# srndpty/kobato-eyes

Measured on AMD Instinct MI355X. Metric: images/s (pHash + all-pairs Hamming scan + cluster membership), higher is better.
Workload: dtype u8 luma, int32 taps (i8 matrix cores), f64 DCT, 1-bit Hamming products (fp4 matrix cores, exact)

## Files before the change

kobato-eyes_amd/csrc/ke_hash.hip:

```cpp
#include <cstdlib>

#include "ke_internal.h"
#include "dct_table.h"
#include "ke_hash_select.h"
#include "ke_resample_plan.h"

namespace {

constexpr int kPrecisionBits = 22;

__device__ __forceinline__ int clip8_fixed(int acc) {
    int v = acc >> kPrecisionBits;
    return v < 0 ? 0 : (v > 255 ? 255 : v);
}

__device__ __forceinline__ int luma_of(const uint8_t *p, int ch) {
    if (ch == 1) return p[0];
    return (int)((19595u * p[0] + 38470u * p[1] + 7471u * p[2] + 0x8000u) >> 16);
}

template <int AXIS>
__global__ __launch_bounds__(256) void ke_resample_pass(const uint8_t *__restrict__ src,
                                                         const uint64_t *__restrict__ offsets, uint64_t stride,
                                                         int ch, int w, int h, const int32_t *__restrict__ bounds,
                                                         const int32_t *__restrict__ kk, int ksize, int out_size,
                                                         uint8_t *__restrict__ dst, int blocks_per_image) {
    const int64_t img = blockIdx.x / blocks_per_image;
    const int blk = blockIdx.x % blocks_per_image;
    const int ow = AXIS == 0 ? out_size : w;
    const int oh = AXIS == 0 ? h : out_size;
    const int e = blk * 256 + threadIdx.x;
    if (e >= ow * oh) return;
    const int oy = e / ow, ox = e % ow;
    const uint8_t *base = src + (offsets ? offsets[img] : (uint64_t)img * stride);
    const int o = AXIS == 0 ? ox : oy;
    const int first = bounds[2 * o], cnt = bounds[2 * o + 1];
    const int32_t *k = kk + (size_t)o * ksize;
    int acc = 1 << (kPrecisionBits - 1);
    if (AXIS == 0) {
        const uint8_t *row = base + ((size_t)oy * w + first) * ch;
        for (int t = 0; t < cnt; ++t) acc += luma_of(row + (size_t)t * ch, ch) * k[t];
    } else {
        const uint8_t *col = base + ((size_t)first * w + ox) * ch;
        for (int t = 0; t < cnt; ++t) acc += luma_of(col + (size_t)t * w * ch, ch) * k[t];
    }
    dst[(size_t)img * ow * oh + e] = (uint8_t)clip8_fixed(acc);
}

__constant__ double c_C32[4][16];
__constant__ double c_C16[2][8];
__constant__ double c_C8[4];

__device__ double dct32_one(const double *x, int k) {
    if (k & 1) {
        const int q = k >> 1;
        double acc = 0.0;
#pragma unroll
        for (int n = 0; n < 16; ++n) acc = fma(x[n] - x[31 - n], c_C32[q][n], acc);
        return acc;
    }
    double u[16];
#pragma unroll
    for (int n = 0; n < 16; ++n) u[n] = x[n] + x[31 - n];
    if (k & 2) {
        const int q = k >> 2;
        double acc = 0.0;
#pragma unroll
        for (int n = 0; n < 8; ++n) acc = fma(u[n] - u[15 - n], c_C16[q][n], acc);
        return acc;
    }
    double v[8];
#pragma unroll
    for (int n = 0; n < 8; ++n) v[n] = u[n] + u[15 - n];
    if (k == 4) {
        double acc = 0.0;
#pragma unroll
        for (int n = 0; n < 4; ++n) acc = fma(v[n] - v[7 - n], c_C8[n], acc);
        return acc;
    }
    const double w0 = v[0] + v[7], w1 = v[1] + v[6], w2 = v[2] + v[5], w3 = v[3] + v[4];
    return (w0 + w1) + (w2 + w3);
}

__device__ uint64_t tile32_to_phash(const uint8_t *tile, double *Td, float *cf, int tid, float *margin = nullptr) {
    {
        const int y = tid >> 3, kx = tid & 7;
        double x[32];
#pragma unroll
        for (int n = 0; n < 32; ++n) x[n] = (double)tile[y * 32 + n];
        Td[y * 8 + kx] = dct32_one(x, kx);
    }
    __syncthreads();
    if (tid < 64) {
        const int ky = tid >> 3, kx = tid & 7;
        double x[32];
#pragma unroll
        for (int n = 0; n < 32; ++n) x[n] = Td[n * 8 + kx];
        const double s = (ky == 0 && kx == 0) ? KE_SCALE00 : ((ky == 0 || kx == 0) ? KE_SCALE0K : KE_SCALEKK);
        cf[tid] = (float)(dct32_one(x, ky) * s);
    }
    __syncthreads();
    uint64_t hash = 0;
    if (tid < 64) {
        const float *a = cf + 1;
        float r[8];
#pragma unroll
        for (int j = 0; j < 8; ++j) r[j] = a[j];
#pragma unroll
        for (int i = 8; i < 56; i += 8)
#pragma unroll
            for (int j = 0; j < 8; ++j) r[j] = r[j] + a[i + j];
        float res = ((r[0] + r[1]) + (r[2] + r[3])) + ((r[4] + r[5]) + (r[6] + r[7]));
#pragma unroll
        for (int i = 56; i < 63; ++i) res = res + a[i];
        const float mean = res / 63.0f;
        const unsigned long long m = __ballot(cf[tid] > mean);
        hash = __brevll(m);
        if (margin) {
            float mg = fabsf(cf[tid] - mean);
#pragma unroll
            for (int s = 32; s > 0; s >>= 1) mg = fminf(mg, __shfl_xor(mg, s));
            if (tid == 0) *margin = mg;
        }
    }
    return hash;
}

__global__ __launch_bounds__(256) void ke_tiles_to_hashes(const uint8_t *__restrict__ tile32,
                                                           const uint8_t *__restrict__ tile98,
                                                           const int64_t *__restrict__ out_idx,
                                                           uint64_t *__restrict__ phash, uint64_t *__restrict__ dhash,
                                                           float *__restrict__ margin) {
    __shared__ __attribute__((aligned(16))) uint8_t s_tile[1024];
    __shared__ double s_T[256];
    __shared__ float s_cf[64];
    const int tid = threadIdx.x;
    const int64_t img = blockIdx.x;
    const int64_t slot = out_idx ? out_idx[img] : img;
    if (phash) {
        reinterpret_cast<uint32_t *>(s_tile)[tid] = reinterpret_cast<const uint32_t *>(tile32 + (size_t)img * 1024)[tid];
        __syncthreads();
        const uint64_t hv = tile32_to_phash(s_tile, s_T, s_cf, tid, margin ? margin + slot : nullptr);
        if (tid == 0) phash[slot] = hv;
    }
    if (dhash && tid < 64) {
        const uint8_t *t = tile98 + (size_t)img * 72;
        const int r = tid >> 3, c = tid & 7;
        const unsigned long long m = __ballot(t[r * 9 + c + 1] > t[r * 9 + c]);
        if (tid == 0) dhash[slot] = __brevll(m);
    }
}

template <bool kTransposed>
__device__ __forceinline__ void tile32_coeffs(const uint8_t *tile, double *Td, float *cf, int tid) {
    {
        const int y = tid >> 3, kx = tid & 7;
        double x[32];
#pragma unroll
        for (int n = 0; n < 32; ++n) x[n] = (double)tile[kTransposed ? n * 32 + y : y * 32 + n];
        Td[y * 8 + kx] = dct32_one(x, kx);
    }
    __syncthreads();
    if (tid < 64) {
        const int ky = tid >> 3, kx = tid & 7;
        double x[32];
#pragma unroll
        for (int n = 0; n < 32; ++n) x[n] = Td[n * 8 + kx];
        const double s = (ky == 0 && kx == 0) ? KE_SCALE00 : ((ky == 0 || kx == 0) ? KE_SCALE0K : KE_SCALEKK);
        cf[tid] = (float)(dct32_one(x, ky) * s);
    }
    __syncthreads();
}

__global__ __launch_bounds__(256) void ke_tiles_to_phash_turned(const uint8_t *__restrict__ tile32, const int64_t *__restrict__ out_idx,
                                                                 uint64_t *__restrict__ turned) {
    __shared__ __attribute__((aligned(16))) uint8_t s_tile[1024];
    __shared__ double s_T[256];
    __shared__ float s_cf[2][64];
    const int tid = threadIdx.x, lane = tid & 63, wv = tid >> 6;
    const int64_t img = blockIdx.x;
    const int64_t slot = out_idx ? out_idx[img] : img;
    reinterpret_cast<uint32_t *>(s_tile)[tid] = reinterpret_cast<const uint32_t *>(tile32 + (size_t)img * 1024)[tid];
    __syncthreads();
    tile32_coeffs<false>(s_tile, s_T, s_cf[0], tid);
// ... 15 lines not shown
#pragma unroll
        for (int i = 56; i < 63; ++i) res = res + coef(1 + i);
        const float mean = res / 63.0f;
        const unsigned long long m = __ballot(coef(lane) > mean);
        if (lane == 0) turned[slot * 8 + k] = __brevll(m);
    }
}

__device__ __forceinline__ uint32_t luma4_biased(uint32_t d0, uint32_t d1, uint32_t d2) {
    constexpr uint32_t CHI = 0x001D964Cu, CLO = 0x002F468Bu, START = 0x8000u - 0x800000u;
    const uint32_t p0 = d0;
    const uint32_t p1 = __builtin_amdgcn_alignbyte(d1, d0, 3);
    const uint32_t p2 = __builtin_amdgcn_alignbyte(d2, d1, 2);
    const uint32_t s0 = (__builtin_amdgcn_udot4(p0, CHI, 0u, false) << 8) + __builtin_amdgcn_udot4(p0, CLO, START, false);
    const uint32_t s1 = (__builtin_amdgcn_udot4(p1, CHI, 0u, false) << 8) + __builtin_amdgcn_udot4(p1, CLO, START, false);
    const uint32_t s2 = (__builtin_amdgcn_udot4(p2, CHI, 0u, false) << 8) + __builtin_amdgcn_udot4(p2, CLO, START, false);
    const uint32_t s3 = (__builtin_amdgcn_udot4(d2, CHI << 8, 0u, false) << 8) + __builtin_amdgcn_udot4(d2, CLO << 8, START, false);
    const uint32_t lo = __builtin_amdgcn_perm(s1, s0, 0x0C0C0602u);
    const uint32_t hi = __builtin_amdgcn_perm(s3, s2, 0x06020C0Cu);
    return lo | hi;
}

template <int C>
__device__ __forceinline__ uint32_t luma4_generic(const uint32_t *d) {
    if (C == 3) return luma4_biased(d[0], d[1], d[2]);
    if (C == 1) return d[0] ^ 0x80808080u;
    constexpr uint32_t CHI = 0x001D964Cu, CLO = 0x002F468Bu, START = 0x8000u - 0x800000u;
    uint32_t s[4];
#pragma unroll
    for (int k = 0; k < 4; ++k)
        s[k] = (__builtin_amdgcn_udot4(d[k], CHI, 0u, false) << 8) + __builtin_amdgcn_udot4(d[k], CLO, START, false);
    return __builtin_amdgcn_perm(s[1], s[0], 0x0C0C0602u) | __builtin_amdgcn_perm(s[3], s[2], 0x06020C0Cu);
}

__device__ __forceinline__ int combine_planes(int d0, int d1, int d2, int bias) {
    return (int)((uint32_t)d0 + ((uint32_t)d1 << 8) + ((uint32_t)d2 << 16) + (uint32_t)bias);
}

struct KeFusedArgs {
    const uint8_t *pixels;
    const uint64_t *offsets;
    uint64_t stride;
    const int64_t *out_idx;
    int h;
    const int32_t *mx_frag;
    int mx_base0, mx_base1;
    const int32_t *h_bias;
    const int32_t *v_packed, *v_start, *v_bias;
    int ndwv;
    int qw, qw_inv, lp;
    int w, row_bytes;
    int lt_half;
    int lt_bytes;
    int hp;
    uint64_t *phash;
    float *margin;
    uint8_t *tile32_out;
    const int32_t *mxd_frag, *hd_bias;
    const int32_t *vd_cpacked, *vd_cstart, *vd_bias;
    int ndwcv;
    int hpd;
    int x_off;
    int bands, band_rows;
    uint8_t *hs, *hsd;
    int hs_hp, hsd_hp;
    uint64_t *dhash;
    uint8_t *tile98_out;
};

template <int C>
__device__ __forceinline__ void patch_last_quad(const uint8_t *image_last_row, int w, uint8_t *lds_row) {
    for (int x = w & ~3; x < w; ++x) lds_row[x] = (uint8_t)(luma_of(image_last_row + (size_t)x * C, C) ^ 0x80);
}

__device__ __forceinline__ void band_writeout(const uint8_t *HT, int hp, int ncols, int rows, uint8_t *dst, int dst_hp, int tid,
                                              int nthreads) {
    const int wpc = (rows + 3) / 4;
    for (int e = tid; e < ncols * wpc; e += nthreads) {
        const int col = e / wpc, k = e % wpc;
        *reinterpret_cast<uint32_t *>(dst + (size_t)col * dst_hp + 4 * k) = *reinterpret_cast<const uint32_t *>(HT + col * hp + 4 * k);
    }
}

template <int NDWD>
__device__ __forceinline__ void fused_tail(const KeFusedArgs &a, uint8_t *Lt, const uint8_t *HT, const uint8_t *HTd,
                                           const int tid, const int64_t img) {
    uint8_t *T32 = Lt;
    double *Td = reinterpret_cast<double *>(Lt + 1024);
    float *cf = reinterpret_cast<float *>(Lt + 1024 + 2048);
    {
        const int yy = tid & 31, og = tid >> 5;
        const int rotv = (yy >> 4) & 1;
        const int vst = a.v_start[yy];
        const int ndwv = a.ndwv;
        int acc[4][3];
#pragma unroll
        for (int m = 0; m < 4; ++m) acc[m][0] = acc[m][1] = acc[m][2] = 0;
        for (int j = 0; j < ndwv; j += 2) {
            const int jj = j ^ (2 * rotv);
            const int32_t *cp = a.v_packed + ((size_t)yy * ndwv + jj) * 3;
            const int c00 = cp[0], c01 = cp[1], c02 = cp[2], c10 = cp[3], c11 = cp[4], c12 = cp[5];
#pragma unroll
            for (int m = 0; m < 4; ++m) {
                const uint2 v = *reinterpret_cast<const uint2 *>(
                    __builtin_assume_aligned(HT + (size_t)(og + 8 * m) * a.hp + vst + 4 * jj, 8));
                acc[m][0] = __builtin_amdgcn_sdot4((int)v.x, c00, acc[m][0], false);
                acc[m][1] = __builtin_amdgcn_sdot4((int)v.x, c01, acc[m][1], false);
                acc[m][2] = __builtin_amdgcn_sdot4((int)v.x, c02, acc[m][2], false);
                acc[m][0] = __builtin_amdgcn_sdot4((int)v.y, c10, acc[m][0], false);
                acc[m][1] = __builtin_amdgcn_sdot4((int)v.y, c11, acc[m][1], false);
                acc[m][2] = __builtin_amdgcn_sdot4((int)v.y, c12, acc[m][2], false);
            }
        }
        const int vbias = a.v_bias[yy];
#pragma unroll
        for (int m = 0; m < 4; ++m)
            T32[yy * 32 + og + 8 * m] = (uint8_t)clip8_fixed(combine_planes(acc[m][0], acc[m][1], acc[m][2], vbias));
    }
    __syncthreads();
    if (a.tile32_out)
        reinterpret_cast<uint32_t *>(a.tile32_out + (size_t)img * 1024)[tid] = reinterpret_cast<const uint32_t *>(T32)[tid];
    const int64_t slot = a.out_idx ? a.out_idx[img] : img;
    const uint64_t hv = tile32_to_phash(T32, Td, cf, tid, (a.margin && a.phash) ? a.margin + slot : nullptr);
    if (tid == 0 && a.phash) a.phash[slot] = hv;
    if (NDWD > 0) {
        __syncthreads();
        int *part = reinterpret_cast<int *>(Lt);
        uint8_t *T98 = Lt + 1024;
        if (tid < 216) {
            const int out = tid / 3, chunk = tid % 3;
            const int yy = out / 9, oc = out % 9;
            const int vc = yy * 3 + chunk;
            const int vst = a.vd_cstart[vc];
            const int nd = a.ndwcv;
            int d0 = 0, d1 = 0, d2 = 0;
            for (int j = 0; j < nd; j += 2) {
                const int32_t *cp = a.vd_cpacked + ((size_t)vc * nd + j) * 3;
                const uint2 v = *reinterpret_cast<const uint2 *>(__builtin_assume_aligned(HTd + (size_t)oc * a.hpd + vst + 4 * j, 8));
                d0 = __builtin_amdgcn_sdot4((int)v.x, cp[0], d0, false);
                d1 = __builtin_amdgcn_sdot4((int)v.x, cp[1], d1, false);
                d2 = __builtin_amdgcn_sdot4((int)v.x, cp[2], d2, false);
                d0 = __builtin_amdgcn_sdot4((int)v.y, cp[3], d0, false);
                d1 = __builtin_amdgcn_sdot4((int)v.y, cp[4], d1, false);
                d2 = __builtin_amdgcn_sdot4((int)v.y, cp[5], d2, false);
            }
            part[tid] = combine_planes(d0, d1, d2, 0);
        }
        __syncthreads();
        if (tid < 72) {
            const int yy = tid / 9;
            const uint32_t sum = (uint32_t)part[3 * tid] + (uint32_t)part[3 * tid + 1] + (uint32_t)part[3 * tid + 2] + (uint32_t)a.vd_bias[yy];
            T98[tid] = (uint8_t)clip8_fixed((int)sum);
        }
        __syncthreads();
        if (a.tile98_out && tid < 72) a.tile98_out[(size_t)img * 72 + tid] = T98[tid];
        if (tid < 64) {
            const int r = tid >> 3, c = tid & 7;
            const unsigned long long m = __ballot(T98[r * 9 + c + 1] > T98[r * 9 + c]);
            if (tid == 0 && a.dhash) a.dhash[a.out_idx ? a.out_idx[img] : img] = __brevll(m);
        }
    }
}

int upload_dct_tables(ke_ctx *ctx) {
    if (ctx->dct_tables_ready) return KE_OK;
    KE_HIP(ctx, hipMemcpyToSymbol(HIP_SYMBOL(c_C32), KE_C32, sizeof(KE_C32)));
    KE_HIP(ctx, hipMemcpyToSymbol(HIP_SYMBOL(c_C16), KE_C16, sizeof(KE_C16)));
    KE_HIP(ctx, hipMemcpyToSymbol(HIP_SYMBOL(c_C8), KE_C8, sizeof(KE_C8)));
    ctx->dct_tables_ready = true;
    return KE_OK;
}

constexpr int kRTM = kKeTileRowsMx;
typedef int ke_v4i __attribute__((ext_vector_type(4)));

template <int W64, int KS, bool DH, bool GEN, int C, bool UNAL>
__global__ __launch_bounds__(256, 2) void ke_phash_fused_mx(const KeFusedArgs a) {
    static_assert(!UNAL || GEN, "rows that are not a multiple of 4 pixels need the run-time row length");
    constexpr uint32_t QB = 4u * C;
    constexpr int W = 64 * W64;
    constexpr int QPT = kRTM * (W / 4) / 256;
    const int QW = GEN ? a.qw : W / 4;
    const int QUADS_PER_TILE = kRTM * QW;
    const int LP = GEN ? a.lp : W + 16;
    constexpr int KD = (W64 + 1) / 2;
    extern __shared__ __attribute__((aligned(16))) uint8_t smem[];
    uint8_t *Lt = smem;
    uint8_t *HT = smem + a.lt_bytes;
    uint8_t *HTd = HT + 32 * a.hp;
    uint8_t *X = smem + a.x_off;
    const int tid = threadIdx.x;
    const int lane = tid & 63, wv = tid >> 6;
    const int64_t img = a.bands ? blockIdx.x / a.bands : blockIdx.x;
    const int y_begin = a.bands ? (int)(blockIdx.x % a.bands) * a.band_rows : 0;
    const uint32_t row_bytes = UNAL ? (uint32_t)a.row_bytes : (uint32_t)QW * QB;
    const uint8_t *src = a.pixels + (a.offsets ? a.offsets[img] : (uint64_t)img * a.stride) + (size_t)y_begin * row_bytes;
    const int h = a.bands ? min(a.band_rows, a.h - y_begin) : a.h;
    const uint32_t image_bytes = (uint32_t)(a.h - y_begin) * row_bytes;

    const int mt = wv >> 1, jt = wv & 1;
    ke_v4i bf[KS][3];
#pragma unroll
    for (int s = 0; s < KS; ++s)
#pragma unroll
        for (int p = 0; p < 3; ++p)
            bf[s][p] = reinterpret_cast<const ke_v4i *>(a.mx_frag)[((jt * KS + s) * 3 + p) * 64 + lane];
    constexpr int KDR = DH ? KD : 1;
    ke_v4i bd[KDR][3];
    int dbias = 0;
    if (DH) {
#pragma unroll
        for (int d = 0; d < KDR; ++d)
#pragma unroll
            for (int p = 0; p < 3; ++p)
                bd[d][p] = reinterpret_cast<const ke_v4i *>(a.mxd_frag)[((jt * KD + d) * 3 + p) * 64 + lane];
        dbias = a.hd_bias[(lane & 15) < 9 ? (lane & 15) : 8];
    }
    const int ocol = 16 * jt + (lane & 15);
    const int hbias = a.h_bias[ocol];
    const int a_off = (16 * mt + (lane & 15)) * LP + (jt ? a.mx_base1 : a.mx_base0) + 16 * (lane >> 4);
    const int d_off = (16 * mt + (lane & 15)) * LP + 64 * KD * jt + 16 * (lane >> 4);
    uint8_t *ht_dst = HT + (size_t)ocol * a.hp + 16 * mt + 4 * (lane >> 4);
    uint8_t *htd_dst = HTd + (size_t)(lane & 15) * a.hpd + 16 * mt + 4 * (lane >> 4);
    ke_v4i *x_slot = reinterpret_cast<ke_v4i *>(X + mt * 1024 + lane * 16);

    uint32_t raw[QPT][C];
    auto load_tile = [&](int t) {
        const uint32_t tile_off = UNAL ? (uint32_t)t * (kRTM * row_bytes) : (uint32_t)t * ((uint32_t)QUADS_PER_TILE * QB);
        const uint8_t *tile_ptr = src + tile_off;
        const uint32_t lim = UNAL ? image_bytes - QB - tile_off : min(image_bytes - QB - tile_off, (uint32_t)(QUADS_PER_TILE - 1) * QB);
#pragma unroll
        for (int q = 0; q < QPT; ++q) {
            uint32_t vo = (uint32_t)(q * 256 + tid) * QB;
            if (UNAL) {
                const uint32_t i = min((uint32_t)(q * 256 + tid), (uint32_t)(QUADS_PER_TILE - 1));
                const uint32_t row = __umulhi(i, (uint32_t)a.qw_inv);
                vo = row * row_bytes + (i - row * (uint32_t)QW) * QB;
            }
            const uint32_t off = vo < lim ? vo : lim;
            const uint32_t *p = reinterpret_cast<const uint32_t *>(tile_ptr + off);
#pragma unroll
            for (int k = 0; k < C; ++k) raw[q][k] = __builtin_nontemporal_load(p + k);
        }
    };
    auto store_luma = [&](uint8_t *dst) {
#pragma unroll
        for (int q = 0; q < QPT; ++q) {
            const int i = q * 256 + tid;
            if (GEN) {
                const int row = (int)__umulhi((uint32_t)i, (uint32_t)a.qw_inv);
                if (i < QUADS_PER_TILE)
                    *reinterpret_cast<uint32_t *>(dst + row * LP + (i - row * QW) * 4) = luma4_generic<C>(raw[q]);
            } else {
                *reinterpret_cast<uint32_t *>(dst + (i / (W / 4)) * LP + (i % (W / 4)) * 4) = luma4_generic<C>(raw[q]);
            }
        }
    };
    auto pack_rows = [](const ke_v4i &v0, const ke_v4i &v1, const ke_v4i &v2, int bias) {
        uint32_t packed = 0;
#pragma unroll
        for (int i = 0; i < 4; ++i) packed |= (uint32_t)clip8_fixed(combine_planes(v0[i], v1[i], v2[i], bias)) << (8 * i);
        return packed ^ 0x80808080u;
    };
    auto products = [&](int t, const uint8_t *cur) -> ke_v4i {
        ke_v4i acc[3], dacc[3];
#pragma unroll
        for (int p = 0; p < 3; ++p) acc[p] = dacc[p] = ke_v4i{0, 0, 0, 0};
        const uint8_t *ap = cur + a_off;
#pragma unroll
        for (int s = 0; s < KS; ++s) {
            const ke_v4i av = *reinterpret_cast<const ke_v4i *>(__builtin_assume_aligned(ap + 64 * s, 16));
#pragma unroll
            for (int p = 0; p < 3; ++p) acc[p] = __builtin_amdgcn_mfma_i32_16x16x64_i8(av, bf[s][p], acc[p], 0, 0, 0);
        }
        if (DH) {
            const uint8_t *dp = cur + d_off;
#pragma unroll
            for (int d = 0; d < KDR; ++d) {
                const ke_v4i av = *reinterpret_cast<const ke_v4i *>(__builtin_assume_aligned(dp + 64 * d, 16));
#pragma unroll
                for (int p = 0; p < 3; ++p) dacc[p] = __builtin_amdgcn_mfma_i32_16x16x64_i8(av, bd[d][p], dacc[p], 0, 0, 0);
            }
        }
        *reinterpret_cast<uint32_t *>(ht_dst + t * kRTM) = pack_rows(acc[0], acc[1], acc[2], hbias);
        ke_v4i part;
#pragma unroll
        for (int i = 0; i < 4; ++i) part[i] = combine_planes(dacc[0][i], dacc[1][i], dacc[2][i], 0);
        return part;
    };
    ke_v4i carry = {0, 0, 0, 0};
    auto finish_dhash = [&](int t) {
        const ke_v4i other = x_slot[(t & 1) * 128];
        const ke_v4i zero = {0, 0, 0, 0};
        const ke_v4i sum = carry + other;
        const uint32_t packed = pack_rows(sum, zero, zero, dbias);
        if ((lane & 15) < 9) *reinterpret_cast<uint32_t *>(htd_dst + t * kRTM) = packed;
    };
    auto hpass = [&](int t, const uint8_t *cur) {
        if (!DH) {
            products(t, cur);
        } else if (jt) {
            x_slot[(t & 1) * 128] = products(t, cur);
        } else {
            if (t > 0) finish_dhash(t - 1);
            carry = products(t, cur);
        }
    };

    const int ntiles = (h + kRTM - 1) / kRTM;
    load_tile(0);
    store_luma(Lt);
    __syncthreads();
    for (int t = 0; t + 1 < ntiles; ++t) {
        load_tile(t + 1);
        __builtin_amdgcn_sched_barrier(0);
        hpass(t, Lt + (t & 1) * a.lt_half);
        __builtin_amdgcn_sched_barrier(0);
        store_luma(Lt + ((t + 1) & 1) * a.lt_half);
        __syncthreads();
    }
    if (UNAL) {
        if (tid == 0 && y_begin + h == a.h)
            patch_last_quad<C>(src + (size_t)(h - 1) * row_bytes, a.w, Lt + ((ntiles - 1) & 1) * a.lt_half + ((h - 1) - (ntiles - 1) * kRTM) * LP);
        __syncthreads();
    }
    hpass(ntiles - 1, Lt + ((ntiles - 1) & 1) * a.lt_half);
    __syncthreads();
    if (DH) {
        if (!jt) finish_dhash(ntiles - 1);
        __syncthreads();
    }
    if (a.bands) {
        band_writeout(HT, a.hp, 32, h, a.hs + (size_t)img * 32 * a.hs_hp + y_begin, a.hs_hp, tid, 256);
        if (DH) band_writeout(HTd, a.hpd, 9, h, a.hsd + (size_t)img * 9 * a.hsd_hp + y_begin, a.hsd_hp, tid, 256);
        return;
    }
    fused_tail<(DH ? 1 : 0)>(a, Lt, HT, HTd, tid, img);
}

constexpr int kRTW = kKeTileRowsWide;

template <int KSH, int QPT, bool DH, int KDW, int C, bool UNAL>
__global__ __launch_bounds__(512, 1) void ke_phash_fused_wide(const KeFusedArgs a) {
    constexpr uint32_t QB = 4u * C;
    extern __shared__ __attribute__((aligned(16))) uint8_t smem[];
    uint8_t *Lt = smem;
    uint8_t *HT = smem + a.lt_bytes;
    uint8_t *HTd = HT + 32 * a.hp;
    uint8_t *X = smem + a.x_off;
    const int tid = threadIdx.x;
    const int lane = tid & 63, wv = tid >> 6;
    const int jt = wv & 1, kh = wv >> 1;
    const int64_t img = a.bands ? blockIdx.x / a.bands : blockIdx.x;
    const int y_begin = a.bands ? (int)(blockIdx.x % a.bands) * a.band_rows : 0;
    const int QW = a.qw, LP = a.lp;
    const uint32_t row_bytes = UNAL ? (uint32_t)a.row_bytes : (uint32_t)QW * QB;
    const uint8_t *src = a.pixels + (a.offsets ? a.offsets[img] : (uint64_t)img * a.stride) + (size_t)y_begin * row_bytes;
    const int h = a.bands ? min(a.band_rows, a.h - y_begin) : a.h;
    const int quads_per_tile = kRTW * QW;
    const uint32_t image_bytes = (uint32_t)(a.h - y_begin) * row_bytes;

    ke_v4i bf[KSH][3];
#pragma unroll
    for (int s = 0; s < KSH; ++s)
#pragma unroll
        for (int p = 0; p < 3; ++p)
            bf[s][p] = reinterpret_cast<const ke_v4i *>(a.mx_frag)[((jt * 4 * KSH + kh * KSH + s) * 3 + p) * 64 + lane];
    const int ocol = 16 * jt + (lane & 15);
    const int hbias = a.h_bias[ocol];
    const int a_off = (lane & 15) * LP + (jt ? a.mx_base1 : a.mx_base0) + 64 * KSH * kh + 16 * (lane >> 4);
    uint8_t *ht_dst = HT + (size_t)ocol * a.hp + 4 * (lane >> 4);
    ke_v4i *x_slot = reinterpret_cast<ke_v4i *>(X) + jt * 192 + lane;
    constexpr int KDR = DH ? KDW : 1;
    ke_v4i bd[KDR][3];
    int dbias = 0;
    if (DH) {
#pragma unroll
        for (int d = 0; d < KDR; ++d)
#pragma unroll
            for (int p = 0; p < 3; ++p)
                bd[d][p] = reinterpret_cast<const ke_v4i *>(a.mxd_frag)[((wv * KDW + d) * 3 + p) * 64 + lane];
        dbias = a.hd_bias[(lane & 15) < 9 ? (lane & 15) : 8];
    }
    const int d_off = (lane & 15) * LP + 64 * KDW * wv + 16 * (lane >> 4);
    uint8_t *htd_dst = HTd + (size_t)(lane & 15) * a.hpd + 4 * (lane >> 4);
    ke_v4i *xd_slot = reinterpret_cast<ke_v4i *>(X) + 768 + lane;

    uint32_t raw[QPT][C];
    auto load_tile = [&](int t) {
        const uint32_t tile_off = UNAL ? (uint32_t)t * (kRTW * row_bytes) : (uint32_t)t * ((uint32_t)quads_per_tile * QB);
        const uint8_t *tile_ptr = src + tile_off;
        const uint32_t lim = UNAL ? image_bytes - QB - tile_off : min(image_bytes - QB - tile_off, (uint32_t)(quads_per_tile - 1) * QB);
#pragma unroll
        for (int q = 0; q < QPT; ++q) {
            uint32_t vo = (uint32_t)(q * 512 + tid) * QB;
            if (UNAL) {
                const uint32_t i = min((uint32_t)(q * 512 + tid), (uint32_t)(quads_per_tile - 1));
                const uint32_t row = __umulhi(i, (uint32_t)a.qw_inv);
                vo = row * row_bytes + (i - row * (uint32_t)QW) * QB;
            }
            const uint32_t off = vo < lim ? vo : lim;
            const uint32_t *p = reinterpret_cast<const uint32_t *>(tile_ptr + off);
#pragma unroll
            for (int c = 0; c < C; ++c) raw[q][c] = __builtin_nontemporal_load(p + c);
        }
    };
    auto store_luma = [&](uint8_t *dst) {
#pragma unroll
        for (int q = 0; q < QPT; ++q) {
            const int i = q * 512 + tid;
            const int row = (int)__umulhi((uint32_t)i, (uint32_t)a.qw_inv);
            if (i < quads_per_tile)
                *reinterpret_cast<uint32_t *>(dst + row * LP + (i - row * QW) * 4) = luma4_generic<C>(raw[q]);
        }
    };
    auto products = [&](const uint8_t *cur) -> ke_v4i {
        ke_v4i acc[3];
#pragma unroll
        for (int p = 0; p < 3; ++p) acc[p] = ke_v4i{0, 0, 0, 0};
        const uint8_t *ap = cur + a_off;
#pragma unroll
        for (int s = 0; s < KSH; ++s) {
            const ke_v4i av = *reinterpret_cast<const ke_v4i *>(__builtin_assume_aligned(ap + 64 * s, 16));
#pragma unroll
            for (int p = 0; p < 3; ++p) acc[p] = __builtin_amdgcn_mfma_i32_16x16x64_i8(av, bf[s][p], acc[p], 0, 0, 0);
        }
        ke_v4i part;
#pragma unroll
        for (int i = 0; i < 4; ++i) part[i] = combine_planes(acc[0][i], acc[1][i], acc[2][i], 0);
        return part;
    };
    auto dproducts = [&](const uint8_t *cur) -> ke_v4i {
        ke_v4i dacc[3];
#pragma unroll
        for (int p = 0; p < 3; ++p) dacc[p] = ke_v4i{0, 0, 0, 0};
        const uint8_t *dp = cur + d_off;
#pragma unroll
        for (int d = 0; d < KDR; ++d) {
            const ke_v4i av = *reinterpret_cast<const ke_v4i *>(__builtin_assume_aligned(dp + 64 * d, 16));
#pragma unroll
            for (int p = 0; p < 3; ++p) dacc[p] = __builtin_amdgcn_mfma_i32_16x16x64_i8(av, bd[d][p], dacc[p], 0, 0, 0);
        }
        ke_v4i part;
#pragma unroll
        for (int i = 0; i < 4; ++i) part[i] = combine_planes(dacc[0][i], dacc[1][i], dacc[2][i], 0);
        return part;
    };
    ke_v4i carry = {0, 0, 0, 0}, dcarry = {0, 0, 0, 0};
    auto dfinish = [&](int t) {
        const ke_v4i *xs = xd_slot + (t & 1) * 448;
        ke_v4i sum = dcarry;
#pragma unroll
        for (int k = 0; k < 7; ++k) sum += xs[64 * k];
        uint32_t packed = 0;
#pragma unroll
        for (int i = 0; i < 4; ++i) packed |= (uint32_t)clip8_fixed((int)((uint32_t)sum[i] + (uint32_t)dbias)) << (8 * i);
        if ((lane & 15) < 9) *reinterpret_cast<uint32_t *>(htd_dst + t * kRTW) = packed ^ 0x80808080u;
    };
    auto finish = [&](int t) {
        const ke_v4i *xs = x_slot + (t & 1) * 384;
        const ke_v4i sum = carry + xs[0] + xs[64] + xs[128];
        uint32_t packed = 0;
#pragma unroll
        for (int i = 0; i < 4; ++i) packed |= (uint32_t)clip8_fixed((int)((uint32_t)sum[i] + (uint32_t)hbias)) << (8 * i);
        *reinterpret_cast<uint32_t *>(ht_dst + t * kRTW) = packed ^ 0x80808080u;
    };
    auto hpass = [&](int t, const uint8_t *cur) {
        if (kh) {
            x_slot[(t & 1) * 384 + (kh - 1) * 64] = products(cur);
        } else {
            if (t > 0) finish(t - 1);
            carry = products(cur);
        }
        if (DH) {
            if (wv) {
                xd_slot[(t & 1) * 448 + (wv - 1) * 64] = dproducts(cur);
            } else {
                if (t > 0) dfinish(t - 1);
                dcarry = dproducts(cur);
            }
        }
    };

    const int ntiles = (h + kRTW - 1) / kRTW;
    load_tile(0);
    store_luma(Lt);
    __syncthreads();
    for (int t = 0; t + 1 < ntiles; ++t) {
        load_tile(t + 1);
        __builtin_amdgcn_sched_barrier(0);
        hpass(t, Lt + (t & 1) * a.lt_half);
        __builtin_amdgcn_sched_barrier(0);
        store_luma(Lt + ((t + 1) & 1) * a.lt_half);
        __syncthreads();
    }
    if (UNAL) {
        if (tid == 0 && y_begin + h == a.h)
            patch_last_quad<C>(src + (size_t)(h - 1) * row_bytes, a.w, Lt + ((ntiles - 1) & 1) * a.lt_half + ((h - 1) - (ntiles - 1) * kRTW) * LP);
        __syncthreads();
    }
    hpass(ntiles - 1, Lt + ((ntiles - 1) & 1) * a.lt_half);
    __syncthreads();
    if (!kh) finish(ntiles - 1);
    if (DH && !wv) dfinish(ntiles - 1);
    __syncthreads();
    if (a.bands) {
        band_writeout(HT, a.hp, 32, h, a.hs + (size_t)img * 32 * a.hs_hp + y_begin, a.hs_hp, tid, 512);
        if (DH) band_writeout(HTd, a.hpd, 9, h, a.hsd + (size_t)img * 9 * a.hsd_hp + y_begin, a.hsd_hp, tid, 512);
        return;
    }
    if (tid >= 256) return;
    fused_tail<(DH ? 1 : 0)>(a, Lt, HT, HTd, tid, img);
}

struct KeBandArgs {
    const uint8_t *pixels;
    const uint64_t *offsets;
    uint64_t stride;
    int w, h;
    int qr;
    int lp;
    int rt;
    int band_rows;
    int bands;
    int nout;
    int nout_total;
    int out_first;
    int cpo_log2;
    int vcp_log2;
    const int32_t *cpacked, *cstart, *cxor, *bias;
    int lt_half;
    int bp;
    uint8_t *hs;
    int hp;
};

template <int NDWC, int C, bool ALIGNED>
__global__ __launch_bounds__(256, 3) void ke_hband(const KeBandArgs a) {
    constexpr int QPT = 8;
    constexpr int DW = C;
    extern __shared__ __attribute__((aligned(16))) uint8_t smem[];
    const int tid = threadIdx.x;
    const int64_t img = blockIdx.x / a.bands;
    const int band = blockIdx.x % a.bands;
    const uint8_t *src = a.pixels + (a.offsets ? a.offsets[img] : (uint64_t)img * a.stride);
    const int y_begin = band * a.band_rows;
    const int y_end = min(a.h, y_begin + a.band_rows);
    const uintptr_t last_dword = ((uintptr_t)src + (uintptr_t)a.w * a.h * C - 1) & ~(uintptr_t)3;

    const int vcl = tid & ((1 << a.vcp_log2) - 1);
    const int rg = tid >> a.vcp_log2, RG = 256 >> a.vcp_log2;
    const int nvc = a.nout << a.cpo_log2;
    const int vloc = vcl < nvc ? vcl : nvc - 1;
    const int o = vloc >> a.cpo_log2;
    const int vc = vloc + (a.out_first << a.cpo_log2);
    const bool writer = vcl < nvc && (vloc & ((1 << a.cpo_log2) - 1)) == 0;
    const int xs = a.cxor[vc];
    int ck[NDWC][3];
#pragma unroll
    for (int p = 0; p < NDWC / 2; ++p)
#pragma unroll
        for (int e = 0; e < 2; ++e)
#pragma unroll
            for (int c = 0; c < 3; ++c) ck[2 * p + e][c] = a.cpacked[((size_t)vc * NDWC + 2 * (p ^ xs) + e) * 3 + c];
    const int cst = a.cstart[vc];
    const int sw[4] = {cst + 8 * (0 ^ xs), cst + 8 * (1 ^ xs), cst + 8 * (2 ^ xs), cst + 8 * (3 ^ xs)};
    const int obias = a.bias[a.out_first + o];

    const int items = a.rt * a.qr;
    const int total_pix = a.w * a.h;
    int rel_pix[QPT], lds_off[QPT];
    {
        int r = tid / a.qr, j = tid % a.qr;
        const int dr = 256 / a.qr, dj = 256 % a.qr;
#pragma unroll
        for (int q = 0; q < QPT; ++q) {
            rel_pix[q] = r * a.w + 4 * j;
            lds_off[q] = (q * 256 + tid < items) ? r * a.lp + 4 * j : -1;
            r += dr; j += dj;
            if (j >= a.qr) { j -= a.qr; ++r; }
        }
    }

    uint32_t raw[QPT][DW];
    const uint32_t image_bytes = (uint32_t)total_pix * C;
    auto load_tile = [&](int ty0) {
        const uint32_t tile_off = (uint32_t)(ty0 * a.w) * C;
        const uint8_t *tile_ptr = src + tile_off;
#pragma unroll
        for (int q = 0; q < QPT; ++q) {
            const uint32_t rel = (uint32_t)rel_pix[q] * C;
            if (ALIGNED) {
                const uint32_t lim = image_bytes - 4u * C - tile_off;
                const uint32_t off = rel < lim ? rel : lim;
                const uint32_t *p = reinterpret_cast<const uint32_t *>(tile_ptr + off);
// ... 707 lines not shown
```

kobato-eyes_amd/csrc/ke_resample_plan.h:

```cpp
#pragma once
#include <algorithm>
#include <cstddef>
#include <cstdint>

#include "ke_coeffs.h"
#include "ke_hash_select.h"

struct KeHashSwitches {
    bool fused_min_set = false;
    int64_t fused_min_images = 0;
    bool vtile_valu = false;
};

struct KePlanShape {
    int w, h, channels;
    int64_t n;
    bool misaligned, base_dword, stride_dword, has_offsets;
};

enum KeDecline {
    KE_PLAN_OK = 0,
    KE_DECLINE_ONE_LAUNCH,
    KE_DECLINE_HB_VERTICAL_FIRST,
    KE_DECLINE_HB_SHAPE,
    KE_DECLINE_HB_WINDOW,
    KE_DECLINE_HB_ROW,
    KE_DECLINE_HB_LDS,
    KE_DECLINE_VT_LDS,
    KE_DECLINE_ST_TARGET,
    KE_DECLINE_ST_SHAPE,
    KE_DECLINE_ST_ADDRESS,
    KE_DECLINE_ST_STEPS,
    KE_DECLINE_ST_TABLE,
    KE_DECLINE_ST_LAST_STRIP,
    KE_DECLINE_ST_SWITCH,
    KE_DECLINE_ST_FILL,
    KE_DECLINE_SPB_SHAPE,
    KE_DECLINE_FU_WIDTH,
    KE_DECLINE_FU_TABLE,
    KE_DECLINE_FU_DH_TABLE,
    KE_DECLINE_FU_LDS,
    KE_DECLINE_FU_BANDS_FIT,
    KE_DECLINE_COUNT
};

inline int ke_column_pitch(int span, int h) { return ((std::max(span, h + 4) + 7) & ~7) + 8; }

inline bool ke_fits_one_launch(int64_t workgroups) { return workgroups <= 0x7fffffffLL; }

inline int64_t ke_chunk_images(size_t per_image) { return std::max<int64_t>(1, (int64_t)(((size_t)512 << 20) / per_image)); }
inline size_t ke_hash_scratch_per_image(int h) { return (size_t)40 * (std::max(h, 32) + 1024); }
inline size_t ke_resize_scratch_per_image(int ow, int oh, int h) { return (size_t)(ow + 8) * (std::max(h, oh) + 1024); }

inline int64_t ke_fused_min_images(int64_t image_bytes, const KeHashSwitches &sw) {
    if (sw.fused_min_set) return sw.fused_min_images;
    return image_bytes < 400 * 1024 ? 1 : image_bytes < (8 << 20) ? 192 : 512;
}

struct KeHbandChunks {
    KeDecline why;
    int best_log2;
};

inline KeHbandChunks ke_plan_hband_chunks(const KePlanShape &g, int ow, int oh, int ndw) {
    if (ke_taller_than_100_widths(g.w, g.h) && oh < g.h) return {KE_DECLINE_HB_VERTICAL_FIRST, -1};
    if ((int64_t)g.w * g.h < 4 || g.w > 16384 || g.h > 65536 || (int64_t)g.w * g.h * g.channels >= (1LL << 31)) return {KE_DECLINE_HB_SHAPE, -1};
    int best_log2 = -1, best_waste = 1 << 30;
    for (int l = 0; l <= 5; ++l) {
        const int cpo = 1 << l, ndwc = (((ndw + cpo - 1) / cpo) + 7) & ~7;
        if (ndwc > 32) continue;
        const int launches = (ow * cpo + 255) / 256;
        const int waste = cpo * ndwc - ndw + (ndwc > 24 ? 8 : 0) + 1000 * (launches - 1);
        if (waste < best_waste) { best_waste = waste; best_log2 = l; }
    }
    if (best_log2 < 0) return {KE_DECLINE_HB_WINDOW, -1};
    return {KE_PLAN_OK, best_log2};
}

struct KeHbandPlan {
    KeDecline why;
    int best_log2;
    int qr, lp, rt, band_rows, bands, bp;
    int per_launch;
    int launches;
    int lt_half, hp;
    size_t lds, scratch_bytes;
    bool aligned;
};
// ... 127 lines not shown
    if (!ke_fits_one_launch((int64_t)g.n * p.bands)) p.why = KE_DECLINE_ONE_LAUNCH;
    return p;
}

struct KeSpBandPlan {
    KeDecline why;
    int bands, band_rows;
    int hs_hp, hsd_hp;
    size_t scratch_bytes;
};

inline KeSpBandPlan ke_plan_sp_bands(const KePlanShape &g, bool want_d, int vspan, int vdspan, int cu_count) {
    KeSpBandPlan p{};
    if (ke_taller_than_100_widths(g.w, g.h) || g.h < 16) { p.why = KE_DECLINE_SPB_SHAPE; return p; }
    const int64_t fill = (4 * (int64_t)cu_count + g.n - 1) / g.n;
    const bool both = want_d && g.channels == 3;
    const int64_t fixed = (g.w <= 768 && !(both && g.w > 512)) ? 64 * (int64_t)(g.w + 32) + (both ? 4096 : 0)
                                                               : 32 * (int64_t)(g.w + 32) + 12288 + (both ? 14336 : 0);
    int64_t max_rows = (80 * 1024 - fixed) / (both ? 41 : 32) / 32 * 32 - 32;
    if (max_rows < 128) max_rows = 1024;
    max_rows = std::min<int64_t>(max_rows, 1024);
    const int64_t bands = std::max<int64_t>((g.h + max_rows - 1) / max_rows, std::min<int64_t>(fill, (g.h + 63) / 64));
    p.band_rows = (int)(((g.h + bands - 1) / bands + 31) / 32 * 32);
    p.bands = (g.h + p.band_rows - 1) / p.band_rows;
    p.hs_hp = ke_column_pitch(vspan, g.h);
    p.hsd_hp = want_d ? ke_column_pitch(vdspan, g.h) : 8;
    p.scratch_bytes = (size_t)g.n * (32 * (size_t)p.hs_hp + (want_d ? 9 * (size_t)p.hsd_hp : 0)) + 8192;
    return p;
}

constexpr int kKeTileRowsMx = 32, kKeTileRowsWide = 16;

struct KeFusedSteps {
    KeDecline why;
    int ks;
    int ksd;
};

inline KeFusedSteps ke_plan_fused_steps(int r, int W) {
    const KeSpRow &row = kKeSpRows[r];
    const bool wide = row.family == KE_SP_WIDE;
    KeFusedSteps s{KE_PLAN_OK, wide ? 4 * row.t[0] : row.t[1], wide ? 8 * row.t[3] : 2 * ((row.t[0] + 1) / 2)};
    if ((W % 4 != 0) != row.unal() || (wide ? kKeTileRowsWide * ((W + 3) / 4) > 512 * row.t[1] : W < row.w_lo || W > row.w_hi)) s.why = KE_DECLINE_FU_WIDTH;
    return s;
}

struct KeFusedPlan {
    KeDecline why;
    int qw, qw_inv, lp, lt_half, hp, hpd, x_off;
    int row_bytes;
    int threads;
    int64_t workgroups;
    size_t lds;
    bool raise_lds_limit;
};

inline KeFusedPlan ke_plan_fused(int r, int W, int h, int64_t n, const KeFusedSteps &s, const KeMxTable &mx, int vspan, const KeMxTable *mxd,
                                 const KeChunkTable *vd, const KeSpBandPlan *bands) {
    const KeSpRow &row = kKeSpRows[r];
    const bool wide = row.family == KE_SP_WIDE, DH = row.dh();
    const int C = row.channels();
    const int rt = wide ? kKeTileRowsWide : kKeTileRowsMx;
    const bool exact = !wide && !row.t[3];
    KeFusedPlan p{};
    p.threads = wide ? 512 : 256;
    if (mx.tiles != 2 || mx.ks != s.ks) { p.why = KE_DECLINE_FU_TABLE; return p; }
    const int rows_padded = bands ? bands->band_rows : ((h + rt - 1) / rt) * rt;
    const int overhang = std::max(0, std::max(std::max(mx.base[0], mx.base[1]) + 64 * s.ks, DH ? 64 * s.ksd : 0) - W);
    p.qw = (W + 3) / 4;
    p.row_bytes = W * C;
    p.qw_inv = (int)(uint32_t)((0x100000000ull + (uint64_t)p.qw - 1) / (uint64_t)p.qw);
    p.lp = exact ? W + 16 : (((W + 15) / 16 + 1) | 1) * 16;
    p.lt_half = (rt * p.lp + overhang + 15) & ~15;
    p.hp = ((std::max(bands ? 0 : vspan, rows_padded) + 7) & ~7) + 8;
    p.hpd = 8;
    p.lds = (size_t)2 * p.lt_half + (size_t)32 * p.hp;
    if (!wide) p.lds = std::max<size_t>(p.lds, 4096);
    if (DH) {
        if (mxd->tiles != 1 || mxd->base[0] != 0 || mxd->ks != s.ksd) { p.why = KE_DECLINE_FU_DH_TABLE; return p; }
        p.hpd = ((std::max(bands ? 0 : vd->cspan, rows_padded) + 7) & ~7) + 8;
        p.lds += (size_t)9 * p.hpd;
    }
    if (wide || DH) {
        p.lds = (p.lds + 15) & ~(size_t)15;
        p.x_off = (int)p.lds;
        p.lds += wide ? 2 * 2 * 3 * 1024 + (DH ? 2 * 7 * 1024 : 0) : 4096;
    }
    if (p.lds > 150 * 1024) { p.why = KE_DECLINE_FU_LDS; return p; }
    if (!bands && p.lds > 80 * 1024 && p.lds - (size_t)(32 * (p.hp - 136)) - (DH ? (size_t)(9 * (p.hpd - 136)) : 0) <= 80 * 1024) { p.why = KE_DECLINE_FU_BANDS_FIT; return p; }
    p.raise_lds_limit = p.lds > 64 * 1024;
    p.workgroups = n * (bands ? bands->bands : 1);
    if (!ke_fits_one_launch(p.workgroups)) p.why = KE_DECLINE_ONE_LAUNCH;
    return p;
}

struct KeGenericPlan {
    bool vertical_first;
    int mid_w, mid_h;
    size_t mid_bytes;
    int64_t max_n;
    int b0, b1;
};

inline KeGenericPlan ke_plan_generic(int w, int h, int ow, int oh) {
    KeGenericPlan p;
    p.vertical_first = ke_taller_than_100_widths(w, h) && oh < h;
    p.mid_w = p.vertical_first ? w : ow;
    p.mid_h = p.vertical_first ? oh : h;
    p.mid_bytes = (size_t)p.mid_w * p.mid_h;
    p.max_n = ke_chunk_images(p.mid_bytes);
    p.b0 = (int)((p.mid_bytes + 255) / 256);
    p.b1 = (ow * oh + 255) / 256;
    return p;
}
```

Baseline: 8.781 million.

## Overlap dHash vertical pass with pHash DCT in fused tail

```diff
diff --git a/kobato-eyes_amd/csrc/ke_dual_tail.h b/kobato-eyes_amd/csrc/ke_dual_tail.h
--- /dev/null
+++ b/kobato-eyes_amd/csrc/ke_dual_tail.h
@@ -0,0 +1,48 @@
+#pragma once
+
+#if defined(__HIPCC__)
+#define KE_DUAL_FN __host__ __device__ inline
+#else
+#define KE_DUAL_FN inline
+#endif
+
+constexpr int kKeDualColumns = 9, kKeDualRows = 8;
+constexpr int kKeDualOutputs = kKeDualRows * kKeDualColumns;
+constexpr int kKeDualChunks = 3;
+constexpr int kKeDualVcols = kKeDualRows * kKeDualChunks;
+constexpr int kKeDualSlices = 8;
+constexpr int kKeDualSums = kKeDualOutputs * kKeDualChunks;
+constexpr int kKeDualTailThreads = 256;
+constexpr int kKeDualFirstThread = 64;
+constexpr int kKeDualWorkers = kKeDualVcols * kKeDualSlices;
+static_assert(kKeDualFirstThread + kKeDualWorkers == kKeDualTailThreads, "waves 1..3 are the workers");
+static_assert(64 % kKeDualSlices == 0, "the slices of a vcol lie in one wave");
+
+constexpr int kKeDualExchangeBytes = 4096;
+constexpr int kKeDualPartOff = 0, kKeDualPartBytes = kKeDualSums * 4;
+constexpr int kKeDualTileOff = 1024, kKeDualTileBytes = kKeDualOutputs;
+static_assert(kKeDualPartOff + kKeDualPartBytes <= kKeDualTileOff, "the sums end in front of the tile");
+static_assert(kKeDualTileOff + kKeDualTileBytes <= kKeDualExchangeBytes, "the scratch fits the exchange buffer");
+
+KE_DUAL_FN int ke_dual_vcol(int output, int chunk) { return (output / kKeDualColumns) * kKeDualChunks + chunk; }
+KE_DUAL_FN int ke_dual_sum_index(int output, int chunk) { return output * kKeDualChunks + chunk; }
+
+KE_DUAL_FN int ke_dual_worker_vcol(int tid) {
+    const int u = tid - kKeDualFirstThread;
+    return u >= 0 && u < kKeDualWorkers ? u / kKeDualSlices : -1;
+}
+KE_DUAL_FN int ke_dual_worker_slice(int tid) {
+    const int u = tid - kKeDualFirstThread;
+    return u >= 0 && u < kKeDualWorkers ? u % kKeDualSlices : -1;
+}
+KE_DUAL_FN int ke_dual_block_slice(int block) { return block % kKeDualSlices; }
+KE_DUAL_FN int ke_dual_vcol_row(int vcol) { return vcol / kKeDualChunks; }
+KE_DUAL_FN int ke_dual_vcol_chunk(int vcol) { return vcol % kKeDualChunks; }
+KE_DUAL_FN bool ke_dual_worker_writes(int tid) { return ke_dual_worker_slice(tid) == 0; }
+
+KE_DUAL_FN int ke_dual_sum_output(int tid) {
+    const int u = tid - kKeDualFirstThread;
+    return u >= 0 && u < kKeDualOutputs ? u : -1;
+}
+
+constexpr int kKeDualBitsFirstThread = 64, kKeDualBitsThreads = 64;
diff --git a/kobato-eyes_amd/csrc/ke_hash.hip b/kobato-eyes_amd/csrc/ke_hash.hip
--- a/kobato-eyes_amd/csrc/ke_hash.hip
+++ b/kobato-eyes_amd/csrc/ke_hash.hip
@@ -2,6 +2,7 @@
 
 #include "ke_internal.h"
 #include "dct_table.h"
+#include "ke_dual_tail.h"
 #include "ke_hash_select.h"
 #include "ke_resample_plan.h"
 
@@ -100,6 +101,52 @@
         cf[tid] = (float)(dct32_one(x, ky) * s);
     }
     __syncthreads();
+    uint64_t hash = 0;
+    if (tid < 64) {
+        const float *a = cf + 1;
+        float r[8];
+#pragma unroll
+        for (int j = 0; j < 8; ++j) r[j] = a[j];
+#pragma unroll
+        for (int i = 8; i < 56; i += 8)
+#pragma unroll
+            for (int j = 0; j < 8; ++j) r[j] = r[j] + a[i + j];
+        float res = ((r[0] + r[1]) + (r[2] + r[3])) + ((r[4] + r[5]) + (r[6] + r[7]));
+#pragma unroll
+        for (int i = 56; i < 63; ++i) res = res + a[i];
+        const float mean = res / 63.0f;
+        const unsigned long long m = __ballot(cf[tid] > mean);
+        hash = __brevll(m);
+        if (margin) {
+            float mg = fabsf(cf[tid] - mean);
+#pragma unroll
+            for (int s = 32; s > 0; s >>= 1) mg = fminf(mg, __shfl_xor(mg, s));
+            if (tid == 0) *margin = mg;
+        }
+    }
+    return hash;
+}
+
+__device__ __forceinline__ void tile32_dct_rows(const uint8_t *tile, double *Td, int tid) {
+    const int y = tid >> 3, kx = tid & 7;
+    double x[32];
+#pragma unroll
+    for (int n = 0; n < 32; ++n) x[n] = (double)tile[y * 32 + n];
+    Td[y * 8 + kx] = dct32_one(x, kx);
+}
+
+__device__ __forceinline__ void tile32_dct_cols(const double *Td, float *cf, int tid) {
+    if (tid < 64) {
+        const int ky = tid >> 3, kx = tid & 7;
+        double x[32];
+#pragma unroll
+        for (int n = 0; n < 32; ++n) x[n] = Td[n * 8 + kx];
+        const double s = (ky == 0 && kx == 0) ? KE_SCALE00 : ((ky == 0 || kx == 0) ? KE_SCALE0K : KE_SCALEKK);
+        cf[tid] = (float)(dct32_one(x, ky) * s);
+    }
+}
+
+__device__ __forceinline__ uint64_t tile32_mean_bits(const float *cf, int tid, float *margin) {
     uint64_t hash = 0;
     if (tid < 64) {
         const float *a = cf + 1;
@@ -281,16 +328,94 @@
     }
 }
 
+typedef int ke_v4i __attribute__((ext_vector_type(4)));
+
+struct KeTailScalars {
+    int v_start, v_bias;
+    int vd_start;
+    int vd_bias;
+};
+
+__device__ __forceinline__ KeTailScalars load_tail_scalars(const KeFusedArgs &a, int tid) {
+    KeTailScalars s;
+    s.v_start = a.v_start[tid & 31];
+    s.v_bias = a.v_bias[tid & 31];
+    const int vcol = ke_dual_worker_vcol(tid);
+    s.vd_start = vcol >= 0 ? a.vd_cstart[vcol] : 0;
+    const int out = ke_dual_sum_output(tid);
+    s.vd_bias = out >= 0 ? a.vd_bias[out / kKeDualColumns] : 0;
+    return s;
+}
+
+struct KeDualBlock {
+    ke_v4i t[3];
+};
+
+__device__ __forceinline__ KeDualBlock load_dual_block(const KeFusedArgs &a, int vcol, int block) {
+    const ke_v4i *p = reinterpret_cast<const ke_v4i *>(
+        __builtin_assume_aligned(a.vd_cpacked + ((size_t)vcol * a.ndwcv + 4 * block) * 3, 16));
+    return KeDualBlock{{p[0], p[1], p[2]}};
+}
+
+__device__ __forceinline__ KeDualBlock load_first_dual_block(const KeFusedArgs &a, int tid) {
+    const int vcol = ke_dual_worker_vcol(tid), slice = ke_dual_worker_slice(tid);
+    if (vcol >= 0 && 4 * slice < a.ndwcv) return load_dual_block(a, vcol, slice);
+    const ke_v4i zero = {0, 0, 0, 0};
+    return KeDualBlock{{zero, zero, zero}};
+}
+
+__device__ __forceinline__ void dual_chunk_sums(const KeFusedArgs &a, const uint8_t *HTd, int tid, int vst, const KeDualBlock &first,
+                                                int *part) {
+    const int vcol = ke_dual_worker_vcol(tid), slice = ke_dual_worker_slice(tid);
+    const int nb = a.ndwcv >> 2;
+    int d[kKeDualColumns][3];
+#pragma unroll
+    for (int oc = 0; oc < kKeDualColumns; ++oc) d[oc][0] = d[oc][1] = d[oc][2] = 0;
+    auto mul = [&](const KeDualBlock &k, int block) {
+#pragma unroll
+        for (int oc = 0; oc < kKeDualColumns; ++oc) {
+            const uint2 *v = reinterpret_cast<const uint2 *>(__builtin_assume_aligned(HTd + (size_t)oc * a.hpd + vst + 16 * block, 8));
+            const uint2 va = v[0], vb = v[1];
+            d[oc][0] = __builtin_amdgcn_sdot4((int)va.x, k.t[0][0], d[oc][0], false);
+            d[oc][1] = __builtin_amdgcn_sdot4((int)va.x, k.t[0][1], d[oc][1], false);
+            d[oc][2] = __builtin_amdgcn_sdot4((int)va.x, k.t[0][2], d[oc][2], false);
+            d[oc][0] = __builtin_amdgcn_sdot4((int)va.y, k.t[0][3], d[oc][0], false);
+            d[oc][1] = __builtin_amdgcn_sdot4((int)va.y, k.t[1][0], d[oc][1], false);
+            d[oc][2] = __builtin_amdgcn_sdot4((int)va.y, k.t[1][1], d[oc][2], false);
+            d[oc][0] = __builtin_amdgcn_sdot4((int)vb.x, k.t[1][2], d[oc][0], false);
+            d[oc][1] = __builtin_amdgcn_sdot4((int)vb.x, k.t[1][3], d[oc][1], false);
+            d[oc][2] = __builtin_amdgcn_sdot4((int)vb.x, k.t[2][0], d[oc][2], false);
+            d[oc][0] = __builtin_amdgcn_sdot4((int)vb.y, k.t[2][1], d[oc][0], false);
+            d[oc][1] = __builtin_amdgcn_sdot4((int)vb.y, k.t[2][2], d[oc][1], false);
+            d[oc][2] = __builtin_amdgcn_sdot4((int)vb.y, k.t[2][3], d[oc][2], false);
+        }
+    };
+    if (slice < nb) {
+        mul(first, slice);
+        for (int block = slice + kKeDualSlices; block < nb; block += kKeDualSlices) mul(load_dual_block(a, vcol, block), block);
+    }
+    const int row = ke_dual_vcol_row(vcol), chunk = ke_dual_vcol_chunk(vcol);
+#pragma unroll
+    for (int oc = 0; oc < kKeDualColumns; ++oc) {
+        uint32_t v = (uint32_t)combine_planes(d[oc][0], d[oc][1], d[oc][2], 0);
+#pragma unroll
+        for (int m = 1; m < kKeDualSlices; m <<= 1) v += (uint32_t)__shfl_xor((int)v, m);
+        if (ke_dual_worker_writes(tid)) part[ke_dual_sum_index(row * kKeDualColumns + oc, chunk)] = (int)v;
+    }
+}
+
 template <int NDWD>
 __device__ __forceinline__ void fused_tail(const KeFusedArgs &a, uint8_t *Lt, const uint8_t *HT, const uint8_t *HTd,
-                                           const int tid, const int64_t img) {
+                                           const int tid, const int64_t img, const KeTailScalars &ts) {
     uint8_t *T32 = Lt;
     double *Td = reinterpret_cast<double *>(Lt + 1024);
     float *cf = reinterpret_cast<float *>(Lt + 1024 + 2048);
+    KeDualBlock first_block;
+    if (NDWD > 0) first_block = load_first_dual_block(a, tid);
     {
         const int yy = tid & 31, og = tid >> 5;
         const int rotv = (yy >> 4) & 1;
-        const int vst = a.v_start[yy];
+        const int vst = NDWD > 0 ? ts.v_start : a.v_start[yy];
         const int ndwv = a.ndwv;
         int acc[4][3];
 #pragma unroll
@@ -311,7 +436,7 @@
                 acc[m][2] = __builtin_amdgcn_sdot4((int)v.y, c12, acc[m][2], false);
             }
         }
-        const int vbias = a.v_bias[yy];
+        const int vbias = NDWD > 0 ? ts.v_bias : a.v_bias[yy];
 #pragma unroll
         for (int m = 0; m < 4; ++m)
             T32[yy * 32 + og + 8 * m] = (uint8_t)clip8_fixed(combine_planes(acc[m][0], acc[m][1], acc[m][2], vbias));
@@ -320,44 +445,33 @@
     if (a.tile32_out)
         reinterpret_cast<uint32_t *>(a.tile32_out + (size_t)img * 1024)[tid] = reinterpret_cast<const uint32_t *>(T32)[tid];
     const int64_t slot = a.out_idx ? a.out_idx[img] : img;
-    const uint64_t hv = tile32_to_phash(T32, Td, cf, tid, (a.margin && a.phash) ? a.margin + slot : nullptr);
-    if (tid == 0 && a.phash) a.phash[slot] = hv;
-    if (NDWD > 0) {
-        __syncthreads();
-        int *part = reinterpret_cast<int *>(Lt);
-        uint8_t *T98 = Lt + 1024;
-        if (tid < 216) {
-            const int out = tid / 3, chunk = tid % 3;
-            const int yy = out / 9, oc = out % 9;
-            const int vc = yy * 3 + chunk;
-            const int vst = a.vd_cstart[vc];
-            const int nd = a.ndwcv;
-            int d0 = 0, d1 = 0, d2 = 0;
-            for (int j = 0; j < nd; j += 2) {
-                const int32_t *cp = a.vd_cpacked + ((size_t)vc * nd + j) * 3;
-                const uint2 v = *reinterpret_cast<const uint2 *>(__builtin_assume_aligned(HTd + (size_t)oc * a.hpd + vst + 4 * j, 8));
-                d0 = __builtin_amdgcn_sdot4((int)v.x, cp[0], d0, false);
-                d1 = __builtin_amdgcn_sdot4((int)v.x, cp[1], d1, false);
-                d2 = __builtin_amdgcn_sdot4((int)v.x, cp[2], d2, false);
-                d0 = __builtin_amdgcn_sdot4((int)v.y, cp[3], d0, false);
-                d1 = __builtin_amdgcn_sdot4((int)v.y, cp[4], d1, false);
-                d2 = __builtin_amdgcn_sdot4((int)v.y, cp[5], d2, false);
-            }
-            part[tid] = combine_planes(d0, d1, d2, 0);
-        }
-        __syncthreads();
-        if (tid < 72) {
-            const int yy = tid / 9;
-            const uint32_t sum = (uint32_t)part[3 * tid] + (uint32_t)part[3 * tid + 1] + (uint32_t)part[3 * tid + 2] + (uint32_t)a.vd_bias[yy];
-            T98[tid] = (uint8_t)clip8_fixed((int)sum);
-        }
-        __syncthreads();
-        if (a.tile98_out && tid < 72) a.tile98_out[(size_t)img * 72 + tid] = T98[tid];
-        if (tid < 64) {
-            const int r = tid >> 3, c = tid & 7;
-            const unsigned long long m = __ballot(T98[r * 9 + c + 1] > T98[r * 9 + c]);
-            if (tid == 0 && a.dhash) a.dhash[a.out_idx ? a.out_idx[img] : img] = __brevll(m);
-        }
+    if (NDWD == 0) {
+        const uint64_t hv = tile32_to_phash(T32, Td, cf, tid, (a.margin && a.phash) ? a.margin + slot : nullptr);
+        if (tid == 0 && a.phash) a.phash[slot] = hv;
+        return;
+    }
+    int *part = reinterpret_cast<int *>(Lt + a.x_off + kKeDualPartOff);
+    uint8_t *T98 = Lt + a.x_off + kKeDualTileOff;
+    if (ke_dual_worker_vcol(tid) >= 0) dual_chunk_sums(a, HTd, tid, ts.vd_start, first_block, part);
+    tile32_dct_rows(T32, Td, tid);
+    __syncthreads();
+    tile32_dct_cols(Td, cf, tid);
+    const int out = ke_dual_sum_output(tid);
+    if (out >= 0) {
+        const uint32_t sum = (uint32_t)part[ke_dual_sum_index(out, 0)] + (uint32_t)part[ke_dual_sum_index(out, 1)] +
+                             (uint32_t)part[ke_dual_sum_index(out, 2)] + (uint32_t)ts.vd_bias;
+        const uint8_t v = (uint8_t)clip8_fixed((int)sum);
+        T98[out] = v;
+        if (a.tile98_out) a.tile98_out[(size_t)img * 72 + out] = v;
+    }
+    __syncthreads();
+    if (tid < 64) {
+        const uint64_t hv = tile32_mean_bits(cf, tid, (a.margin && a.phash) ? a.margin + slot : nullptr);
+        if (tid == 0 && a.phash) a.phash[slot] = hv;
+    } else if (tid < kKeDualBitsFirstThread + kKeDualBitsThreads) {
+        const int b = tid - kKeDualBitsFirstThread, r = b >> 3, c = b & 7;
+        const unsigned long long m = __ballot(T98[r * 9 + c + 1] > T98[r * 9 + c]);
+        if (b == 0 && a.dhash) a.dhash[slot] = __brevll(m);
     }
 }
 
@@ -371,7 +485,6 @@
 }
 
 constexpr int kRTM = kKeTileRowsMx;
-typedef int ke_v4i __attribute__((ext_vector_type(4)));
 
 template <int W64, int KS, bool DH, bool GEN, int C, bool UNAL>
 __global__ __launch_bounds__(256, 2) void ke_phash_fused_mx(const KeFusedArgs a) {
@@ -523,18 +636,20 @@
             patch_last_quad<C>(src + (size_t)(h - 1) * row_bytes, a.w, Lt + ((ntiles - 1) & 1) * a.lt_half + ((h - 1) - (ntiles - 1) * kRTM) * LP);
         __syncthreads();
     }
+    KeTailScalars ts{};
+    if (DH && !a.bands) ts = load_tail_scalars(a, tid);
     hpass(ntiles - 1, Lt + ((ntiles - 1) & 1) * a.lt_half);
     __syncthreads();
     if (DH) {
         if (!jt) finish_dhash(ntiles - 1);
-        __syncthreads();
+        if (a.bands) __syncthreads();
     }
     if (a.bands) {
         band_writeout(HT, a.hp, 32, h, a.hs + (size_t)img * 32 * a.hs_hp + y_begin, a.hs_hp, tid, 256);
         if (DH) band_writeout(HTd, a.hpd, 9, h, a.hsd + (size_t)img * 9 * a.hsd_hp + y_begin, a.hsd_hp, tid, 256);
         return;
     }
-    fused_tail<(DH ? 1 : 0)>(a, Lt, HT, HTd, tid, img);
+    fused_tail<(DH ? 1 : 0)>(a, Lt, HT, HTd, tid, img, ts);
 }
 
 constexpr int kRTW = kKeTileRowsWide;
@@ -698,6 +813,8 @@
             patch_last_quad<C>(src + (size_t)(h - 1) * row_bytes, a.w, Lt + ((ntiles - 1) & 1) * a.lt_half + ((h - 1) - (ntiles - 1) * kRTW) * LP);
         __syncthreads();
     }
+    KeTailScalars ts{};
+    if (DH && !a.bands) ts = load_tail_scalars(a, tid);
     hpass(ntiles - 1, Lt + ((ntiles - 1) & 1) * a.lt_half);
     __syncthreads();
     if (!kh) finish(ntiles - 1);
@@ -709,7 +826,7 @@
         return;
     }
     if (tid >= 256) return;
-    fused_tail<(DH ? 1 : 0)>(a, Lt, HT, HTd, tid, img);
+    fused_tail<(DH ? 1 : 0)>(a, Lt, HT, HTd, tid, img, ts);
 }
 
 struct KeBandArgs {
diff --git a/kobato-eyes_amd/csrc/ke_resample_plan.h b/kobato-eyes_amd/csrc/ke_resample_plan.h
--- a/kobato-eyes_amd/csrc/ke_resample_plan.h
+++ b/kobato-eyes_amd/csrc/ke_resample_plan.h
@@ -4,6 +4,7 @@
 #include <cstdint>
 
 #include "ke_coeffs.h"
+#include "ke_dual_tail.h"
 #include "ke_hash_select.h"
 
 struct KeHashSwitches {
@@ -297,9 +298,12 @@
         p.lds += (size_t)9 * p.hpd;
     }
     if (wide || DH) {
+        constexpr int kWidePhashExchange = 2 * 2 * 3 * 1024, kWideDhashExchange = 2 * 7 * 1024;
+        static_assert(kKeDualTileOff + kKeDualTileBytes <= kKeDualExchangeBytes && kKeDualExchangeBytes <= kWidePhashExchange,
+                      "the dHash tail's scratch fits the exchange area of both kernels");
         p.lds = (p.lds + 15) & ~(size_t)15;
         p.x_off = (int)p.lds;
-        p.lds += wide ? 2 * 2 * 3 * 1024 + (DH ? 2 * 7 * 1024 : 0) : 4096;
+        p.lds += wide ? kWidePhashExchange + (DH ? kWideDhashExchange : 0) : kKeDualExchangeBytes;
     }
     if (p.lds > 150 * 1024) { p.why = KE_DECLINE_FU_LDS; return p; }
     if (!bands && p.lds > 80 * 1024 && p.lds - (size_t)(32 * (p.hp - 136)) - (DH ? (size_t)(9 * (p.hpd - 136)) : 0) <= 80 * 1024) { p.why = KE_DECLINE_FU_BANDS_FIT; return p; }
```

After: 8.784 million (median of 4 runs). Within noise of the previous version (+0.0%).
